# KwangsungKim138/Korean-F5-TTS

Measured on AMD Instinct MI355X. Metric: RTF (audio_sec/wall_sec) F5-TTS Base NFE=16 batch=1, higher is better.
Workload: dtype f16; 1 GPU; C2: F5-TTS Base, 1 utterance/rank/step, prompt 256 + generated 768 mel frames, NFE=16 EPSS, cfg 2.0, sway -1, Vocos decode, mel all_gather when n_gpus>1; global_batch=1, frames=1024, parallelism=dp1, weights=synthetic random-init seed 0

## Files before the change

### korean-f5-tts_amd/csrc/gemm2.h

```cpp
#pragma once
#include "gemm.h"


namespace f5 {

template <int N> __device__ __forceinline__ void wait_vmcnt() { asm volatile("s_waitcnt vmcnt(%0)" ::"n"(N) : "memory"); }

__device__ __forceinline__ void glds16(const void* gsrc, char* lds_dst) {
    __builtin_amdgcn_global_load_lds((const __attribute__((address_space(1))) void*)gsrc,
                                     (__attribute__((address_space(3))) void*)lds_dst, 16, 0, 0);
}

__device__ __forceinline__ void lds_read_b128_asm(u32x4& dst, unsigned addr) {
    asm volatile("ds_read_b128 %0, %1" : "=v"(dst) : "v"(addr));
}
template <int N> __device__ __forceinline__ void wait_lgkm(u32x4& a) { asm volatile("s_waitcnt lgkmcnt(%1)" : "+v"(a) : "n"(N > 15 ? 15 : N)); }
template <int N> __device__ __forceinline__ void wait_lgkm(u32x4& a, u32x4& b) {
    asm volatile("s_waitcnt lgkmcnt(%2)" : "+v"(a), "+v"(b) : "n"(N > 15 ? 15 : N));
}
template <int N> __device__ __forceinline__ void wait_lgkm(u32x4& a, u32x4& b, u32x4& c) {
    asm volatile("s_waitcnt lgkmcnt(%3)" : "+v"(a), "+v"(b), "+v"(c) : "n"(N > 15 ? 15 : N));
}
template <int N> __device__ __forceinline__ void wait_lgkm(u32x4& a, u32x4& b, u32x4& c, u32x4& d) {
    asm volatile("s_waitcnt lgkmcnt(%4)" : "+v"(a), "+v"(b), "+v"(c), "+v"(d) : "n"(N > 15 ? 15 : N));
}
template <int N> __device__ __forceinline__ void wait_lgkm(u32x4& a, u32x4& b, u32x4& c, u32x4& d, u32x4& e) {
    asm volatile("s_waitcnt lgkmcnt(%5)" : "+v"(a), "+v"(b), "+v"(c), "+v"(d), "+v"(e) : "n"(N > 15 ? 15 : N));
}

template <int R, int MI, int NJ, int KK, int I>
__device__ __forceinline__ void wait_row_ct(u32x4 (&af)[2][MI], u32x4 (&wf)[2][NJ]) {
    constexpr int idx = KK * (MI + NJ) + NJ + I;
    constexpr int allow = R - 1 - idx;
    if constexpr (I == 0) {
        if constexpr (NJ == 1) wait_lgkm<allow>(af[KK][0], wf[KK][0]);
        else if constexpr (NJ == 2) wait_lgkm<allow>(af[KK][0], wf[KK][0], wf[KK][1]);
        else if constexpr (NJ == 3) wait_lgkm<allow>(af[KK][0], wf[KK][0], wf[KK][1], wf[KK][2]);
        else wait_lgkm<allow>(af[KK][0], wf[KK][0], wf[KK][1], wf[KK][2], wf[KK][3]);
    } else {
        wait_lgkm<allow>(af[KK][I]);
    }
}
template <int R, int MI, int NJ>
__device__ __forceinline__ void wait_row(int kk, int i, u32x4 (&af)[2][MI], u32x4 (&wf)[2][NJ]) {
#define F5_WR(KK, I) if (kk == KK && i == I) { if constexpr (I < MI) wait_row_ct<R, MI, NJ, KK, I>(af, wf); }
    F5_WR(0, 0) F5_WR(0, 1) F5_WR(0, 2) F5_WR(0, 3) F5_WR(0, 4) F5_WR(0, 5) F5_WR(0, 6) F5_WR(0, 7)
    F5_WR(1, 0) F5_WR(1, 1) F5_WR(1, 2) F5_WR(1, 3) F5_WR(1, 4) F5_WR(1, 5) F5_WR(1, 6) F5_WR(1, 7)
#undef F5_WR
}

typedef __attribute__((ext_vector_type(2))) float f32x2_t;
typedef __attribute__((ext_vector_type(2))) _Float16 f16x2_t;
__device__ __forceinline__ void split8_f16(const u32x4& c0, const u32x4& c1, f16x8& hi, f16x8& lo) {
    const f32x4 x0 = __builtin_bit_cast(f32x4, c0), x1 = __builtin_bit_cast(f32x4, c1);
#pragma unroll
    for (int p = 0; p < 4; ++p) {
        const f32x2_t v = p < 2 ? f32x2_t{x0[2 * p], x0[2 * p + 1]} : f32x2_t{x1[2 * p - 4], x1[2 * p - 3]};
        const f16x2_t h = __builtin_convertvector(v, f16x2_t);
        const f32x2_t r = v - __builtin_convertvector(h, f32x2_t);
        const f16x2_t l = __builtin_convertvector(r, f16x2_t);
        hi[2 * p] = h[0]; hi[2 * p + 1] = h[1];
        lo[2 * p] = l[0]; lo[2 * p + 1] = l[1];
    }
}
__device__ __forceinline__ void tie(u32x4& a) { asm volatile("" : "+v"(a)); }

struct GemmConv { int tpt = 0, dil = 0, half = 0, m_base = 0; };

template <typename T, int BM, int BN, int WM, int WN, int NS, typename Epi, int MODE = 0>
__device__ __forceinline__ void gemm_tn_glds_body(char* smem, const T* __restrict__ A, int lda, const T* __restrict__ W,
                                                  int ldw, int M, int N, int K, const Epi& epi, int xa, int xb,
                                                  const int* __restrict__ m_limit, const GemmConv cv = GemmConv{}) {
    constexpr int NW = WM * WN;
    constexpr int KT = GEMM_ROW_BYTES / sizeof(T);
    constexpr int EPC = 16 / sizeof(T);
    constexpr int TM = BM / WM, TN = BN / WN;
    constexpr int MI = TM / 16, NJ = TN / 16;
    constexpr int STAGE = (BM + BN) * GEMM_ROW_BYTES;
    constexpr int RG_A = BM / 8, RG_W = BN / 8;
    constexpr int LA = RG_A / NW, LW = RG_W / NW;
    static_assert(RG_A % NW == 0 && RG_W % NW == 0, "tile rows must split evenly over the waves");
    constexpr int L = LA + LW;

    const int tid = threadIdx.x, lane = tid & 63;
    const int wave = __builtin_amdgcn_readfirstlane(tid >> 6);
    const int wr = wave / WN, wc = wave % WN;
    int tile_m = blockIdx.y, tile_n = blockIdx.x;
    if (m_limit) {
        const int tiles_n = gridDim.x;
        const int bid = blockIdx.y * tiles_n + blockIdx.x;
        const int idx = bid >> 3;
        tile_m = (idx / tiles_n) * 8 + (bid & 7);
        tile_n = idx % tiles_n;
    } else if (xa > 0) {
        const int tiles_n = gridDim.x;
        const int bid = blockIdx.y * tiles_n + blockIdx.x;
        const int xcd = bid & 7, idx = bid >> 3;
        const int rects_n = tiles_n / xb;
        const int per_rect = xa * xb;
        const int rect = xcd + 8 * (idx / per_rect), in = idx % per_rect;
        tile_m = (rect / rects_n) * xa + in / xb;
        tile_n = (rect % rects_n) * xb + in % xb;
    }
    const int m0 = tile_m * BM, n0 = tile_n * BN;
    if (m_limit) {
        M = min(M, __builtin_amdgcn_readfirstlane(*m_limit));
        if (m0 >= M) return;
    }
    const int nkt = K / KT;
    bool trj[NJ];
    int nt = 0;
#pragma unroll
    for (int j = 0; j < NJ; ++j) {
        trj[j] = Epi::kTransposes && epi.tile_transposed(n0 + (wave % WN) * TN + j * 16);
        nt += trj[j] ? 1 : 0;
    }
    nt = __builtin_amdgcn_readfirstlane(nt);

    const int lr = lane >> 3, lc = (lane & 7) ^ lr;
    const T* asrc[LA];
    const T* wsrc[LW];
#pragma unroll
    for (int i = 0; i < LA; ++i) {
        const int row = min(m0 + (wave + i * NW) * 8 + lr, M - 1);
        asrc[i] = A + (size_t)row * lda + lc * EPC;
    }
#pragma unroll
    for (int i = 0; i < LW; ++i) {
        const int row = min(n0 + (wave + i * NW) * 8 + lr, N - 1);
        wsrc[i] = W + (size_t)row * ldw + lc * EPC;
    }
    auto issue_piece = [&](int p, long akoff, int koff, char* base) {
        if (p < LA) glds16(asrc[p] + akoff, base + (wave + p * NW) * 1024);
        else glds16(wsrc[p - LA] + koff, base + BM * GEMM_ROW_BYTES + (wave + (p - LA) * NW) * 1024);
    };
    auto issue = [&](int kt, int stage) {
        if (kt >= nkt) return;
        char* base = smem + stage * STAGE;
        const int koff = kt * KT;
        long akoff = koff;
        if (cv.tpt > 0) {
            const int tap = kt / cv.tpt;
            akoff = (long)(tap - cv.half) * cv.dil * lda + (long)(kt - tap * cv.tpt) * KT;
        }
#pragma unroll
        for (int p = 0; p < L; ++p) issue_piece(p, akoff, koff, base);
    };
    auto wait_tiles = [&](int tiles) {
        if (tiles >= NS - 2) wait_vmcnt<(NS - 2) * L>();
        else if (NS >= 4 && tiles == NS - 3) wait_vmcnt<(NS >= 4 ? NS - 3 : 0) * L>();
        else if (NS >= 5 && tiles == NS - 4) wait_vmcnt<(NS >= 5 ? NS - 4 : 0) * L>();
        else wait_vmcnt<0>();
// ... 40 lines not shown
        if (any_tr) {
#pragma unroll
            for (int i = 0; i < MI; ++i) {
                const int m = min(mw + i * 16 + g * 4, M - 1);
                trc[i] = epi.trow(m + cv.m_base, M + cv.m_base);
            }
#pragma unroll
            for (int j = 0; j < NJ; ++j) tcc[j] = epi.tcol(min(nw + j * 16 + l15, N - 1));
        }
    };
#pragma unroll
    for (int t = 0; t < NS - 1; ++t) issue(t, t);
    if (EARLY) epilogue_setup();

    __builtin_amdgcn_s_waitcnt(0xC07F);
    auto kloop = [&](auto ntc) {
        constexpr int NT = decltype(ntc)::value;
        constexpr int R = 2 * (MI + NJ);
        auto tile = [&](int stage) {
            u32x4 af[2][MI], wf[2][NJ];
            const unsigned sbu = (unsigned)(stage * STAGE) + lds_base;
#pragma unroll
            for (int kk = 0; kk < 2; ++kk) {
                const unsigned co = kk ? c1 : c0;
                lds_read_b128_asm(af[kk][0], sbu + a_row_off + co);
#pragma unroll
                for (int j = 0; j < NJ; ++j) lds_read_b128_asm(wf[kk][j], sbu + w_row_off + j * 16 * GEMM_ROW_BYTES + co);
#pragma unroll
                for (int i = 1; i < MI; ++i) lds_read_b128_asm(af[kk][i], sbu + a_row_off + i * 16 * GEMM_ROW_BYTES + co);
            }
            if constexpr (MODE == 3 || MODE >= 5) {
#pragma unroll
                for (int i = 0; i < MI; ++i) {
                    __builtin_amdgcn_sched_barrier(0);
                    wait_row<R, MI, NJ>(1, i, af, wf);
                    tie(af[0][i]);
                    if (i == 0) {
#pragma unroll
                        for (int j = 0; j < NJ; ++j) tie(wf[0][j]);
                    }
                    f16x8 ah, al;
                    if constexpr (MODE == 5) { ah = __builtin_bit_cast(f16x8, af[0][i]); al = __builtin_bit_cast(f16x8, af[1][i]); }
                    else split8_f16(af[0][i], af[1][i], ah, al);
#pragma unroll
                    for (int term = (MODE == 6 ? 1 : MODE == 7 ? 2 : 0); term < 3; ++term) {
#pragma unroll
                        for (int j = 0; j < NJ; ++j) {
                            const f16x8 w = __builtin_bit_cast(f16x8, wf[term == 0 ? 1 : 0][j]);
                            const f16x8 a = term == 1 ? al : ah;
                            if (j < NJ - NT) acc[i][j] = __builtin_amdgcn_mfma_f32_16x16x32_f16(w, a, acc[i][j], 0, 0, 0);
                            else acc[i][j] = __builtin_amdgcn_mfma_f32_16x16x32_f16(a, w, acc[i][j], 0, 0, 0);
                        }
                    }
                }
                return;
            }
#pragma unroll
            for (int kk = 0; kk < 2; ++kk) {
#pragma unroll
                for (int i = 0; i < MI; ++i) {
                    __builtin_amdgcn_sched_barrier(0);
                    wait_row<R, MI, NJ>(kk, i, af, wf);
#pragma unroll
                    for (int j = 0; j < NJ; ++j) {
                        if (j < NJ - NT) acc[i][j] = Mma<T>::run(wf[kk][j], af[kk][i], acc[i][j]);
                        else acc[i][j] = Mma<T>::run(af[kk][i], wf[kk][j], acc[i][j]);
                    }
                }
            }
        };
        int stage = 0;
        {
            for (int kt = 0; kt < nkt; ++kt) {
                if (MODE != 2) wait_tiles(nkt - 1 - kt);
                __builtin_amdgcn_s_barrier();
                int pf = stage + NS - 1;
                if (pf >= NS) pf -= NS;
                if (MODE != 2) issue(kt + NS - 1, pf);
                if (MODE != 1) tile(stage);
                stage = stage + 1 == NS ? 0 : stage + 1;
            }
        }
    };
    if constexpr (Epi::kTransposes) {
        constexpr bool MIXED = (BN % 64) != 0 || BN == 192;
        if (nt == 0) kloop(std::integral_constant<int, 0>{});
        else if (nt == NJ) kloop(std::integral_constant<int, NJ>{});
        else if constexpr (MIXED && NJ >= 2) {
            if (nt == 1) kloop(std::integral_constant<int, 1>{});
            else if constexpr (NJ >= 3) {
                if (nt == 2) kloop(std::integral_constant<int, 2>{});
                else if constexpr (NJ >= 4) kloop(std::integral_constant<int, 3>{});
            }
        }
    } else {
        kloop(std::integral_constant<int, 0>{});
    }

    if (MODE == 4 && K > 0) {
        float sink = 0.f;
#pragma unroll
        for (int i = 0; i < MI; ++i)
#pragma unroll
            for (int j = 0; j < NJ; ++j) sink += acc[i][j][0] + acc[i][j][1] + acc[i][j][2] + acc[i][j][3];
        if (sink == 1234.5678f && lda < 0) *reinterpret_cast<volatile float*>(smem) = sink;
        return;
    }
    if (!EARLY) epilogue_setup();
    __builtin_amdgcn_s_waitcnt(0x0F70);
#pragma unroll
    for (int j = 0; j < NJ; ++j) {
        const int n = nw + j * 16 + g * 4;
        if (trj[j] || n >= N) continue;
#pragma unroll
        for (int i = 0; i < MI; ++i)
            if (mw + i * 16 + l15 < M) epi.store(rc[i], cc[j], acc[i][j], pre[i][j]);
    }
    if (any_tr) {
#pragma unroll
        for (int j = 0; j < NJ; ++j) {
            const int n = nw + j * 16 + l15;
            if (!trj[j] || n >= N) continue;
#pragma unroll
            for (int i = 0; i < MI; ++i)
                if (mw + i * 16 + g * 4 < M) epi.tstore(trc[i], tcc[j], acc[i][j]);
        }
    }
}

template <typename T, int BM, int BN, int WM, int WN, int NS, typename Epi, int MODE = 0>
__global__ __launch_bounds__(WM* WN * 64) void gemm_tn_glds_kernel(const T* __restrict__ A, int lda,
                                                                   const T* __restrict__ W, int ldw, int M, int N, int K,
                                                                   Epi epi, int xa, int xb, const int* __restrict__ m_limit,
                                                                   const GemmConv cv) {
    extern __shared__ __attribute__((aligned(16))) char smem[];
    gemm_tn_glds_body<T, BM, BN, WM, WN, NS, Epi, MODE>(smem, A, lda, W, ldw, M, N, K, epi, xa, xb, m_limit, cv);
}

inline int& xcd_mode() { static int m = 1; return m; }
inline void pick_xcd_rect(int tiles_m, int tiles_n, int* xa, int* xb) {
    *xa = *xb = 0;
    if (!xcd_mode()) return;
    long best = -1;
    for (int a = 1; a <= tiles_m && a <= 16; ++a) {
        if (tiles_m % a) continue;
        for (int b = 1; b <= tiles_n && b <= 32; ++b) {
            if (tiles_n % b) continue;
            const long rects = (long)(tiles_m / a) * (tiles_n / b);
            if (rects % 8) continue;
            const int area = a * b;
            if (area > 64) continue;
            const long score = 1000L * (64 - (area > 32 ? area - 32 : 32 - area)) - 10L * (a + b);
            if (score > best) { best = score; *xa = a; *xb = b; }
        }
    }
    if (*xa * *xb <= 1) *xa = *xb = 0;
}

template <typename T, int BM, int BN, int WM, int WN, int NS, typename Epi, int MODE = 0>
inline hipError_t launch_gemm2_raw(hipStream_t s, const T* A, int lda, const T* W, int ldw, int M, int N, int K,
                                   const Epi& epi, const int* m_limit = nullptr, const GemmConv& cv = GemmConv{}) {
    constexpr int smem = NS * (BM + BN) * GEMM_ROW_BYTES;
    static bool attr_set = false;
    if (!attr_set) {
        hipError_t e = hipFuncSetAttribute(reinterpret_cast<const void*>(&gemm_tn_glds_kernel<T, BM, BN, WM, WN, NS, Epi, MODE>),
                                           hipFuncAttributeMaxDynamicSharedMemorySize, smem);
        if (e != hipSuccess) return e;
        attr_set = true;
    }
    dim3 grid((N + BN - 1) / BN, (M + BM - 1) / BM);
    if (m_limit) grid.y = (grid.y + 7) / 8 * 8;
    int xa = 0, xb = 0;
    if (!m_limit) pick_xcd_rect((int)grid.y, (int)grid.x, &xa, &xb);
    hipLaunchKernelGGL((gemm_tn_glds_kernel<T, BM, BN, WM, WN, NS, Epi, MODE>), grid, dim3(WM * WN * 64), smem, s, A, lda, W,
                       ldw, M, N, K, epi, xa, xb, m_limit, cv);
    return hipGetLastError();
}

template <typename T, int BM, int BN, int WM, int WN, int NS, typename Epi, int MODE = 0>
inline hipError_t launch_gemm2_cfg(hipStream_t s, const T* A, int lda, const T* W, int ldw, int M, int N, int K,
                                   const Epi& epi, const int* m_limit = nullptr, const GemmConv& cv = GemmConv{}) {
    return with_static_act(epi, [&](const auto& e) {
        return launch_gemm2_raw<T, BM, BN, WM, WN, NS, std::decay_t<decltype(e)>, MODE>(s, A, lda, W, ldw, M, N, K, e, m_limit, cv);
    });
}

}
```

### korean-f5-tts_amd/csrc/gemm3.h

```cpp
#pragma once
#include "gemm2.h"

namespace f5 {

template <typename E, typename = void> struct epi_staged : std::false_type {};
template <typename E> struct epi_staged<E, std::void_t<decltype(E::kStaged)>> : std::integral_constant<bool, E::kStaged> {};

template <int OFF> __device__ __forceinline__ void lds_read_b128_off(u32x4& dst, unsigned addr) {
    asm volatile("ds_read_b128 %0, %1 offset:%2" : "=v"(dst) : "v"(addr), "n"(OFF));
}
__device__ __forceinline__ void reg_fence(u32x4& a) { asm volatile("" : "+v"(a)); }

template <typename T, typename Epi, int DIAG = 0>
__global__ __launch_bounds__(512) void gemm_pp_kernel(const T* __restrict__ A, int lda, const T* __restrict__ W, int ldw, int M,
                                                      int N, int K, Epi epi, int xa, int xb, const int* __restrict__ m_limit) {
    extern __shared__ __attribute__((aligned(16))) char smem[];
    constexpr int BM = 256, BN = 256;
    constexpr int KT = GEMM_ROW_BYTES / sizeof(T);
    constexpr int EPC = 16 / sizeof(T);
    constexpr int MI = 8, NJ = 4;
    constexpr int RB = GEMM_ROW_BYTES;
    constexpr int BUF = (BM + BN) * RB;

    const int tid = threadIdx.x, lane = tid & 63;
    const int wave = __builtin_amdgcn_readfirstlane(tid >> 6);
    const int wr = wave >> 2, wc = wave & 3;
    int tile_m = blockIdx.y, tile_n = blockIdx.x;
    if (m_limit) {
        const int tiles_n = gridDim.x;
        const int bid = blockIdx.y * tiles_n + blockIdx.x;
        const int idx = bid >> 3;
        tile_m = (idx / tiles_n) * 8 + (bid & 7);
        tile_n = idx % tiles_n;
    } else if (xa > 0) {
        const int tiles_n = gridDim.x;
        const int bid = blockIdx.y * tiles_n + blockIdx.x;
        const int xcd = bid & 7, idx = bid >> 3;
        const int rects_n = tiles_n / xb;
        const int per_rect = xa * xb;
        const int rect = xcd + 8 * (idx / per_rect), in = idx % per_rect;
        tile_m = (rect / rects_n) * xa + in / xb;
        tile_n = (rect % rects_n) * xb + in % xb;
    }
    const int m0 = tile_m * BM, n0 = tile_n * BN;
    if (m_limit) {
        M = min(M, __builtin_amdgcn_readfirstlane(*m_limit));
        if (m0 >= M) return;
    }
    const int nkt = K / KT;
    const bool transposed = Epi::kTransposes && epi.tile_transposed(n0);

    const int lr = lane >> 3, lc = (lane & 7) ^ lr;
    const T* asrc[2][2];
    const T* bsrc[2][2];
    int adst[2][2], bdst[2][2];
#pragma unroll
    for (int u = 0; u < 2; ++u)
#pragma unroll
        for (int h = 0; h < 2; ++h) {
            const int ar = h * 128 + u * 64 + wave * 8;
            asrc[u][h] = A + (size_t)min(m0 + ar + lr, M - 1) * lda + lc * EPC;
            adst[u][h] = ar * RB;
            const int q = wave + 8 * h;
            const int br = (q >> 2) * 64 + u * 32 + (q & 3) * 8;
            bsrc[u][h] = W + (size_t)min(n0 + br + lr, N - 1) * ldw + lc * EPC;
            bdst[u][h] = (BM + br) * RB;
        }
    auto issue_a = [&](int u, int koff, char* base) {
        glds16(asrc[u][0] + koff, base + adst[u][0]);
        glds16(asrc[u][1] + koff, base + adst[u][1]);
    };
    auto issue_b = [&](int u, int koff, char* base) {
        glds16(bsrc[u][0] + koff, base + bdst[u][0]);
        glds16(bsrc[u][1] + koff, base + bdst[u][1]);
    };

    f32x4 acc[MI][NJ];
#pragma unroll
    for (int i = 0; i < MI; ++i)
#pragma unroll
        for (int j = 0; j < NJ; ++j) acc[i][j] = f32x4{0.f, 0.f, 0.f, 0.f};

    const int l15 = lane & 15, g = lane >> 4, sw = l15 & 7;
    const unsigned lds_base = (unsigned)(size_t)(__attribute__((address_space(3))) char*)smem;
    const unsigned a_row = (wr * 128 + l15) * RB, b_row = (BM + wc * 64 + l15) * RB;
    const unsigned c0 = ((0 + g) ^ sw) * 16, c1 = ((4 + g) ^ sw) * 16;

    issue_a(0, 0, smem);
    issue_b(0, 0, smem);
    issue_b(1, 0, smem);
    issue_a(1, 0, smem);
    __builtin_amdgcn_s_waitcnt(0xC07F);
    wait_vmcnt<0>();
// ... 211 lines not shown
```

### korean-f5-tts_amd/csrc/gemm_dispatch.h

```cpp
#pragma once
#include "gemm3.h"

namespace f5 {

enum GemmCfg { G2_128x128_8W = 2, G2_128x64_8W = 9, G2_64x64_4W = 8, G2_128x192_8W = 10, G2_256x128_8W = 13, G3_256x256_PP = 20 };

inline int pick_cfg_v2(int M, int N, bool allow_v3 = false, float g3_penalty = 0.f) {
    static const int forced = getenv("F5_GEMM_CFG") ? atoi(getenv("F5_GEMM_CFG")) : -1;
    static const int forced_n = getenv("F5_GEMM_CFG_N") ? atoi(getenv("F5_GEMM_CFG_N")) : 0;
    if (forced >= 0 && (forced != G3_256x256_PP || allow_v3) && (forced_n == 0 || forced_n == N)) return forced;
    if (M <= 64) return G2_64x64_4W;
    struct Cand { int id, bm, bn; float t; };
    static const Cand cands[] = {{G3_256x256_PP, 256, 256, 37.0f}, {G2_256x128_8W, 256, 128, 21.0f}, {G2_128x192_8W, 128, 192, 19.3f},
                                 {G2_128x128_8W, 128, 128, 14.5f}, {G2_128x64_8W, 128, 64, 7.3f}, {G2_64x64_4W, 64, 64, 4.0f}};
    int best = G2_64x64_4W;
    float best_cost = 3.0e38f;
    for (const Cand& c : cands) {
        if (c.id == G3_256x256_PP && !allow_v3) continue;
        const long tiles = (long)((M + c.bm - 1) / c.bm) * ((N + c.bn - 1) / c.bn);
        const float cost = (float)((tiles + 255) / 256) * (c.t + (c.id == G3_256x256_PP ? g3_penalty : 0.f));
        if (cost < best_cost) { best_cost = cost; best = c.id; }
    }
    return best;
}

template <typename Epi> inline bool epilogue_streams_residual(const Epi&) { return false; }
inline bool epilogue_streams_residual(const EpiGateRes&) { return true; }

template <typename T, typename Epi>
inline hipError_t launch_gemm_v2(hipStream_t s, const T* A, int lda, const T* W, int ldw, int M, int N, int K,
                                 const Epi& epi, int cfg, const int* ml = nullptr, const GemmConv& cv = GemmConv{}, int split = 0) {
    if constexpr (std::is_same_v<T, float>) {
        if (split == 2) {
            switch (cfg) {
                case G3_256x256_PP:
                    if (cv.tpt == 0 && cv.m_base == 0) return launch_gemm3<T, Epi, 8>(s, A, lda, W, ldw, M, N, K, epi, ml);
                    [[fallthrough]];
                case G2_256x128_8W: return launch_gemm2_cfg<T, 256, 128, 4, 2, 3, Epi, 5>(s, A, lda, W, ldw, M, N, K, epi, ml, cv);
                case G2_128x192_8W: return launch_gemm2_cfg<T, 128, 192, 2, 4, 3, Epi, 5>(s, A, lda, W, ldw, M, N, K, epi, ml, cv);
                case G2_128x128_8W: return launch_gemm2_cfg<T, 128, 128, 2, 4, 4, Epi, 5>(s, A, lda, W, ldw, M, N, K, epi, ml, cv);
                case G2_128x64_8W: return launch_gemm2_cfg<T, 128, 64, 4, 2, 4, Epi, 5>(s, A, lda, W, ldw, M, N, K, epi, ml, cv);
                default: return launch_gemm2_cfg<T, 64, 64, 2, 2, 3, Epi, 5>(s, A, lda, W, ldw, M, N, K, epi, ml, cv);
            }
        }
        if (split) {
            switch (cfg) {
                case G3_256x256_PP:
                case G2_256x128_8W: return launch_gemm2_cfg<T, 256, 128, 4, 2, 3, Epi, 3>(s, A, lda, W, ldw, M, N, K, epi, ml, cv);
                case G2_128x192_8W: return launch_gemm2_cfg<T, 128, 192, 2, 4, 3, Epi, 3>(s, A, lda, W, ldw, M, N, K, epi, ml, cv);
                case G2_128x128_8W: return launch_gemm2_cfg<T, 128, 128, 2, 4, 4, Epi, 3>(s, A, lda, W, ldw, M, N, K, epi, ml, cv);
                case G2_128x64_8W: return launch_gemm2_cfg<T, 128, 64, 4, 2, 4, Epi, 3>(s, A, lda, W, ldw, M, N, K, epi, ml, cv);
                default: return launch_gemm2_cfg<T, 64, 64, 2, 2, 3, Epi, 3>(s, A, lda, W, ldw, M, N, K, epi, ml, cv);
            }
        }
    } else if (split) return hipErrorInvalidValue;
    switch (cfg) {
        case G3_256x256_PP:
            if (cv.tpt == 0 && cv.m_base == 0) return launch_gemm3<T, Epi>(s, A, lda, W, ldw, M, N, K, epi, ml);
            [[fallthrough]];
        case G2_256x128_8W: return launch_gemm2_cfg<T, 256, 128, 4, 2, 3, Epi>(s, A, lda, W, ldw, M, N, K, epi, ml, cv);
        case G2_128x192_8W: return launch_gemm2_cfg<T, 128, 192, 2, 4, 3, Epi>(s, A, lda, W, ldw, M, N, K, epi, ml, cv);
        case G2_128x128_8W: return launch_gemm2_cfg<T, 128, 128, 2, 4, 4, Epi>(s, A, lda, W, ldw, M, N, K, epi, ml, cv);
        case G2_128x64_8W: return launch_gemm2_cfg<T, 128, 64, 4, 2, 4, Epi>(s, A, lda, W, ldw, M, N, K, epi, ml, cv);
        default: return launch_gemm2_cfg<T, 64, 64, 2, 2, 3, Epi>(s, A, lda, W, ldw, M, N, K, epi, ml, cv);
    }
}

template <typename T, typename Epi>
inline hipError_t launch_gemm(hipStream_t s, const T* A, int lda, const T* W, int ldw, int M, int N, int K,
                              const Epi& epi, int force_cfg = -1, const int* m_limit = nullptr, int m_hint = 0,
                              const GemmConv& cv = GemmConv{}, int split = 0) {
    if (M <= 0 || N <= 0) return hipSuccess;
    if (split && (K % (GEMM_ROW_BYTES / (int)sizeof(T)) != 0 || force_cfg == -2)) return hipErrorInvalidValue;
    constexpr int KT = GEMM_ROW_BYTES / (int)sizeof(T);
    if (cv.tpt > 0 && (K % KT != 0 || force_cfg == -2)) return hipErrorInvalidValue;
    const float g3_pen = 0.0f;
    const bool v3_ok = ((sizeof(T) == 2 && !split) || split == 2) && gemm3_epilogue_ok(epi);
    if (K % KT == 0 && force_cfg == -1 && !m_limit && cv.tpt == 0 && v3_ok) {
        const int rem = M % 256, main = M - rem;
        const int cfg_main = (rem > 0 && rem <= 64 && main >= 4096) ? pick_cfg_v2(main, N, true, g3_pen) : -1;
        if (cfg_main == G3_256x256_PP || cfg_main == G2_256x128_8W) {
            hipError_t e = launch_gemm_v2<T, Epi>(s, A, lda, W, ldw, main, N, K, epi, cfg_main, nullptr, GemmConv{}, split);
            if (e != hipSuccess) return e;
            GemmConv tail{};
            tail.m_base = main;
            return launch_gemm_v2<T, Epi>(s, A + (size_t)main * lda, lda, W, ldw, rem, N, K, epi, G2_64x64_4W, nullptr, tail, split);
        }
    }
    if (K % KT == 0 && force_cfg != -2) {
        int cfg = force_cfg >= 0 ? force_cfg : pick_cfg_v2(m_hint > 0 ? m_hint : M, N, v3_ok && cv.tpt == 0, g3_pen);
        if (split == 2 && force_cfg < 0 && cfg == G2_128x64_8W && (long)((M + 63) / 64) * ((N + 63) / 64) <= 512) cfg = G2_64x64_4W;
        return launch_gemm_v2<T, Epi>(s, A, lda, W, ldw, M, N, K, epi, cfg, m_limit, cv, split);
    }
    if (m_limit) return hipErrorInvalidValue;
    return launch_gemm_v1<T, Epi>(s, A, lda, W, ldw, M, N, K, epi);
}

}
```

### korean-f5-tts_amd/csrc/kapi.hip

```cpp
#include <vector>

#include "attn2.h"
#include "convpos.h"
#include "elementwise.h"
#include "gemm_dispatch.h"
#include "internal.h"

using namespace f5;
#define fail f5_fail
#define F5K_BY_PREC(prec, FN, ...) \
    ((prec) == F5_PREC_BF16 ? FN<bf16_t>(__VA_ARGS__) : (prec) == F5_PREC_F16 ? FN<f16_t>(__VA_ARGS__) : FN<float>(__VA_ARGS__))
static bool g_split16 = false;
template <typename T> static hipError_t maybe_split(hipStream_t s, T* w, size_t elems) {
    if constexpr (std::is_same_v<T, float>) {
        if (g_split16) hipLaunchKernelGGL(split_planar_kernel, dim3(ew_blocks((long)(elems / 32))), dim3(256), 0, s, w, (long)(elems / 32));
    }
    return hipGetLastError();
}

template <typename T>
static int gemm_impl(const float* A, const float* W, const float* bias, int act, float* out, int M, int N, int K, int tm,
                     int tn, hipStream_t s) {
    const int Kp = tm > 0 ? round_up(K, 8) : round_up(K, 128 / (int)sizeof(T));
    Scratch<T> a, w;
// ... 257 lines not shown
                    EpiQKV<TO>{q, k, static_cast<TO*>(p.out2), bias, frag.p, p.Nseq, p.Npad, p.H, norm ? 0 : p.pe_heads,
                               norm ? 1.0f : p.q_scale, rowmap.p},
                    p.cfg, ml, split));
    if (norm) {
        const long qrows = (long)p.Bp * p.H * p.Nseq;
        hipLaunchKernelGGL((qknorm_rope_kernel<TO>), dim3((unsigned)((qrows * 16 + 255) / 256)), dim3(256), 0, s, q, k, p.gq, p.gk,
                           p.rope_cos, p.rope_sin, qrows, p.Nseq, p.H, p.pe_heads, p.q_scale, 1e-6f);
        KCHK();
    }
    CHK(copy_f32<TO>(s, p.out0, p.out0_f32, p.n0));
    CHK(copy_f32<TO>(s, p.out1, p.out1_f32, p.n1));
    CHK(copy_f32<TO>(s, p.out2, p.out2_f32, p.n2));
    HIPCHK(hipStreamSynchronize(s));
    return F5_OK;
}

template <typename T>
static int gemm_epi_impl(const float* A, const float* W, const float* bias, int M, int N, int K, const f5k_epi& p, hipStream_t s) {
    const int Kp = round_up(K, GEMM_ROW_BYTES / (int)sizeof(T));
    Scratch<T> a, w;
    HIPCHK(a.alloc((size_t)M * Kp));
    HIPCHK(w.alloc((size_t)N * Kp));
    hipLaunchKernelGGL((cast_pad_kernel<T>), dim3(ew_blocks((long)M * Kp)), dim3(256), 0, s, A, K, M, K, a.p, Kp, M);
    hipLaunchKernelGGL((cast_pad_kernel<T>), dim3(ew_blocks((long)N * Kp)), dim3(256), 0, s, W, K, N, K, w.p, Kp, N);
    KCHK();
    int split = 0;
    if constexpr (std::is_same_v<T, float>) {
        if (g_split16) {
            HIPCHK(maybe_split<T>(s, w.p, (size_t)N * Kp));
            if (p.a_presplit) HIPCHK(maybe_split<T>(s, a.p, (size_t)M * Kp));
            split = p.a_presplit ? 2 : 1;
        }
    }
    Scratch<int> ml;
    if (p.m_limit >= 0) {
        HIPCHK(ml.alloc(1));
        HIPCHK(hipMemcpy(ml.p, &p.m_limit, 4, hipMemcpyHostToDevice));
    }
    Scratch<int> lens;
    switch (p.kind) {
        case F5K_EPI_STORE:
            if (p.out16) {
                if constexpr (sizeof(T) == 2) {
                    CHK(epi_gemm<T>(s, a.p, w.p, Kp, M, N, Kp, EpiStore<T>{static_cast<T*>(p.out0), N, bias, p.act}, p.cfg, ml.p, split));
                    CHK(copy_f32<T>(s, p.out0, p.out0_f32, p.n0));
                }
            } else {
                CHK(epi_gemm<T>(s, a.p, w.p, Kp, M, N, Kp, EpiStore<float>{static_cast<float*>(p.out0), N, bias, p.act, p.planar == 1}, p.cfg,
                                ml.p, split));
                if (p.planar == 2) {
                    hipLaunchKernelGGL(split_planar_kernel, dim3(ew_blocks((long)M * N / 32)), dim3(256), 0, s, static_cast<float*>(p.out0),
                                       (long)M * N / 32);
                    KCHK();
                }
            }
            break;
        case F5K_EPI_GATE_RES:
            if (p.lens_host) {
                HIPCHK(lens.alloc((size_t)p.nlens));
                HIPCHK(hipMemcpy(lens.p, p.lens_host, (size_t)p.nlens * 4, hipMemcpyHostToDevice));
            }
            CHK(epi_gemm<T>(s, a.p, w.p, Kp, M, N, Kp,
                            EpiGateRes{static_cast<float*>(p.out0), p.res, N, bias, p.gate, p.gate_stride, p.rows_per_batch, lens.p}, p.cfg,
                            ml.p, split));
            break;
        default:
            if (p.out16) {
                if constexpr (std::is_same_v<T, float>) CHK((epi_qkv<T, f16_t>(s, a.p, w.p, Kp, M, N, Kp, bias, p, ml.p, split)));
            } else {
                CHK((epi_qkv<T, T>(s, a.p, w.p, Kp, M, N, Kp, bias, p, ml.p, split)));
            }
            break;
    }
    HIPCHK(hipStreamSynchronize(s));
    return F5_OK;
}

extern "C" int f5k_gemm_epi(int32_t prec, const float* A, const float* W, const float* bias, int32_t M, int32_t N, int32_t K,
                            const f5k_epi* p, f5_stream stream) {
    if (!A || !W || !p || !p->out0 || M <= 0 || N <= 0 || K <= 0 || (N % 4)) return fail(F5_EINVAL, "f5k_gemm_epi: bad arguments (N %% 4 == 0)");
    if (prec != F5_PREC_F32 && prec != F5_PREC_F16X3 && prec != F5_PREC_BF16 && prec != F5_PREC_F16)
        return fail(F5_EINVAL, "f5k_gemm_epi: precision must be f32, f16x3, bf16 or f16");
    const int c = p->cfg;
    if (c != -1 && c != G2_128x128_8W && c != G2_64x64_4W && c != G2_128x64_8W && c != G2_128x192_8W && c != G2_256x128_8W && c != G3_256x256_PP)
        return fail(F5_EINVAL, "f5k_gemm_epi: cfg must be -1, 2, 8, 9, 10, 13 or 20");
    if (p->m_limit < -1 || p->m_limit > M) return fail(F5_EINVAL, "f5k_gemm_epi: m_limit must be -1 or 0..M");
    if (p->a_presplit && prec != F5_PREC_F16X3) return fail(F5_EINVAL, "f5k_gemm_epi: a_presplit needs F5_PREC_F16X3");
    const bool op16 = prec == F5_PREC_BF16 || prec == F5_PREC_F16;
    switch (p->kind) {
        case F5K_EPI_STORE:
            if (p->out16 && !op16) return fail(F5_EINVAL, "f5k_gemm_epi: a 16-bit STORE needs a 16-bit operand precision");
            if (p->planar < 0 || p->planar > 2 || (p->planar && (p->out16 || prec != F5_PREC_F16X3 || N % 32)) || (p->planar == 2 && p->m_limit >= 0))
                return fail(F5_EINVAL, "f5k_gemm_epi: planar needs an f32 output under f16x3 and N %% 32 == 0 (planar 2: every row)");
            if (p->act != F5_ACT_NONE && p->act != F5_ACT_GELU_TANH) return fail(F5_EINVAL, "f5k_gemm_epi: act must be none or GELU-tanh");
            break;
        case F5K_EPI_GATE_RES:
            if (p->out16 || p->rows_per_batch <= 0 || !p->res) return fail(F5_EINVAL, "f5k_gemm_epi: GATE_RES needs res and rows_per_batch > 0");
            if (p->lens_host && p->nlens < (M - 1) / p->rows_per_batch + 1) return fail(F5_EINVAL, "f5k_gemm_epi: lens shorter than the batch rows");
            break;
        case F5K_EPI_QKV:
        case F5K_EPI_QKNORM: {
            const bool norm = p->kind == F5K_EPI_QKNORM;
            if (!p->out1 || !p->out2 || !bias || !p->rope_cos || !p->rope_sin || p->H <= 0 || N != 3 * p->H * 64 || p->Nseq <= 0 ||
                p->Npad < p->Nseq || p->Npad % 8 || p->pe_heads < 0 || p->pe_heads > p->H || p->maxpos < p->Nseq || p->Bp <= 0)
                return fail(F5_EINVAL, "f5k_gemm_epi: bad QKV arguments");
            if (p->out16 && op16) return fail(F5_EINVAL, "f5k_gemm_epi: out16 QKV is the f16 output of f32 / f16x3 operands");
            if (norm && (p->out16 || !p->gq || !p->gk || p->row_start_host)) return fail(F5_EINVAL, "f5k_gemm_epi: bad QKNORM arguments");
            if (p->row_start_host) {
                if (p->m_limit != -1 || p->row_start_host[0] != 0 || p->row_start_host[p->Bp] > M)
                    return fail(F5_EINVAL, "f5k_gemm_epi: row_start must start at 0, end <= M and replaces m_limit");
                for (int b = 0; b < p->Bp; ++b) {
                    const int cnt = p->row_start_host[b + 1] - p->row_start_host[b];
                    if (p->row_start_host[b] % 4 || cnt < 0 || cnt > round_up(p->Nseq, 4))
                        return fail(F5_EINVAL, "f5k_gemm_epi: row_start entries must be multiples of 4, at most round_up(Nseq, 4) apart");
                }
            } else if (M != p->Bp * p->Nseq) {
                return fail(F5_EINVAL, "f5k_gemm_epi: M must be Bp * Nseq without row_start");
            }
            break;
        }
        default: return fail(F5_EINVAL, "f5k_gemm_epi: unknown epilogue kind");
    }
    hipStream_t s = (hipStream_t)stream;
    g_split16 = prec == F5_PREC_F16X3;
    const int rc = F5K_BY_PREC(prec, gemm_epi_impl, A, W, bias, M, N, K, *p, s);
    g_split16 = false;
    return rc;
}
```

### korean-f5-tts_amd/csrc/kapi_diag.hip

```cpp
#include <vector>

#include "attn2.h"
#include "convpos.h"
#include "elementwise.h"
#include "gemm_dispatch.h"
#include "internal.h"

using namespace f5;
#define fail f5_fail
#define F5K_BY_PREC(prec, FN, ...) \
    ((prec) == F5_PREC_BF16 ? FN<bf16_t>(__VA_ARGS__) : (prec) == F5_PREC_F16 ? FN<f16_t>(__VA_ARGS__) : FN<float>(__VA_ARGS__))

#include "gemm2.h"
static int g_cold_weights = 0;
static int g_out_bf16 = 0;

template <typename T, typename Epi>
static hipError_t gemm2_dispatch(int cfg, hipStream_t s, const T* A, int lda, const T* W, int ldw, int M, int N, int K,
                                 const Epi& epi) {
    switch (cfg) {
        case 0: return launch_gemm2_cfg<T, 128, 128, 2, 2, 3, Epi>(s, A, lda, W, ldw, M, N, K, epi);
        case 1: return launch_gemm2_cfg<T, 128, 128, 2, 2, 4, Epi>(s, A, lda, W, ldw, M, N, K, epi);
        case 13: return launch_gemm2_cfg<T, 256, 128, 4, 2, 3, Epi>(s, A, lda, W, ldw, M, N, K, epi);
        case 20: return launch_gemm3<T, Epi>(s, A, lda, W, ldw, M, N, K, epi);
        case 420: return launch_gemm3<T, Epi, 4>(s, A, lda, W, ldw, M, N, K, epi);
        case 2: return launch_gemm2_cfg<T, 128, 128, 2, 4, 4, Epi>(s, A, lda, W, ldw, M, N, K, epi);
        case 3: return launch_gemm2_cfg<T, 128, 64, 2, 2, 4, Epi>(s, A, lda, W, ldw, M, N, K, epi);
        case 5: return launch_gemm2_cfg<T, 64, 64, 2, 2, 4, Epi>(s, A, lda, W, ldw, M, N, K, epi);
        case 7: return launch_gemm2_cfg<T, 128, 128, 4, 2, 3, Epi>(s, A, lda, W, ldw, M, N, K, epi);
        case 8: return launch_gemm2_cfg<T, 64, 64, 2, 2, 3, Epi>(s, A, lda, W, ldw, M, N, K, epi);
        case 9: return launch_gemm2_cfg<T, 128, 64, 4, 2, 4, Epi>(s, A, lda, W, ldw, M, N, K, epi);
        case 10: return launch_gemm2_cfg<T, 128, 192, 2, 4, 3, Epi>(s, A, lda, W, ldw, M, N, K, epi);
        case 11: return launch_gemm2_cfg<T, 128, 192, 2, 4, 4, Epi>(s, A, lda, W, ldw, M, N, K, epi);
        case 102: return launch_gemm2_cfg<T, 128, 128, 2, 4, 4, Epi, 1>(s, A, lda, W, ldw, M, N, K, epi);
        case 202: return launch_gemm2_cfg<T, 128, 128, 2, 4, 4, Epi, 2>(s, A, lda, W, ldw, M, N, K, epi);
        case 16: return launch_gemm2_cfg<T, 128, 128, 2, 4, 2, Epi>(s, A, lda, W, ldw, M, N, K, epi);
        case 17: return launch_gemm2_cfg<T, 256, 128, 4, 2, 2, Epi>(s, A, lda, W, ldw, M, N, K, epi);
        case 18: return launch_gemm2_cfg<T, 128, 128, 2, 2, 2, Epi>(s, A, lda, W, ldw, M, N, K, epi);
        case 113: return launch_gemm2_cfg<T, 256, 128, 4, 2, 3, Epi, 1>(s, A, lda, W, ldw, M, N, K, epi);
        case 213: return launch_gemm2_cfg<T, 256, 128, 4, 2, 3, Epi, 2>(s, A, lda, W, ldw, M, N, K, epi);
        case 413: return launch_gemm2_cfg<T, 256, 128, 4, 2, 3, Epi, 4>(s, A, lda, W, ldw, M, N, K, epi);
        case 402: return launch_gemm2_cfg<T, 128, 128, 2, 4, 4, Epi, 4>(s, A, lda, W, ldw, M, N, K, epi);
        case 409: return launch_gemm2_cfg<T, 128, 64, 4, 2, 4, Epi, 4>(s, A, lda, W, ldw, M, N, K, epi);
        default: return hipErrorInvalidValue;
    }
}

template <typename T>
static int gemm2_impl(const float* A, const float* W, const float* bias, int act, float* out, int M, int N, int K, int cfg,
                      int iters, float* avg_us, hipStream_t s) {
    const int Kp = round_up(K, 128 / (int)sizeof(T));
    Scratch<T> a, w;
    HIPCHK(a.alloc((size_t)M * Kp));
    HIPCHK(w.alloc((size_t)N * Kp));
    hipLaunchKernelGGL((cast_pad_kernel<T>), dim3(ew_blocks((long)M * Kp)), dim3(256), 0, s, A, K, M, K, a.p, Kp, M);
    hipLaunchKernelGGL((cast_pad_kernel<T>), dim3(ew_blocks((long)N * Kp)), dim3(256), 0, s, W, K, N, K, w.p, Kp, N);
    KCHK();
    HIPCHK(gemm2_dispatch<T>(cfg, s, a.p, Kp, w.p, Kp, M, N, Kp, EpiStore<float>{out, N, bias, act}));
    if (iters > 0 && avg_us) {
        const bool cold = g_cold_weights != 0;
        const size_t wbytes = (size_t)N * Kp * sizeof(T);
        const int ncopy = cold ? (int)std::min<size_t>(64, (320u << 20) / wbytes + 1) : 1;
        Scratch<T> wc;
        if (cold) {
            HIPCHK(wc.alloc((size_t)ncopy * N * Kp));
            for (int c = 0; c < ncopy; ++c)
                HIPCHK(hipMemcpyAsync(wc.p + (size_t)c * N * Kp, w.p, wbytes, hipMemcpyDeviceToDevice, s));
        }
        hipEvent_t e0, e1;
        HIPCHK(hipEventCreate(&e0));
        HIPCHK(hipEventCreate(&e1));
        for (int i = 0; cold && i < ncopy; ++i)
            HIPCHK(gemm2_dispatch<T>(cfg, s, a.p, Kp, wc.p + (size_t)(i % ncopy) * N * Kp, Kp, M, N, Kp, EpiStore<float>{out, N, bias, act}));
        HIPCHK(hipEventRecord(e0, s));
        for (int i = 0; i < iters; ++i) {
            const T* wp = cold ? wc.p + (size_t)(i % ncopy) * N * Kp : w.p;
            if (g_out_bf16)
                HIPCHK(gemm2_dispatch<T>(cfg, s, a.p, Kp, wp, Kp, M, N, Kp, EpiStore<bf16_t>{reinterpret_cast<bf16_t*>(out), N, bias, act}));
            else
                HIPCHK(gemm2_dispatch<T>(cfg, s, a.p, Kp, wp, Kp, M, N, Kp, EpiStore<float>{out, N, bias, act}));
        }
        HIPCHK(hipEventRecord(e1, s));
        HIPCHK(hipEventSynchronize(e1));
        float ms = 0.f;
        HIPCHK(hipEventElapsedTime(&ms, e0, e1));
        *avg_us = ms * 1000.f / iters;
        (void)hipEventDestroy(e0);
        (void)hipEventDestroy(e1);
    }
    HIPCHK(hipStreamSynchronize(s));
    return F5_OK;
}

extern "C" int f5x_set_xcd_mode(int32_t on) { xcd_mode() = on; return 0; }
extern "C" int f5x_set_attn_variant(int32_t v) { attn2_variant() = v; return 0; }
extern "C" int f5x_set_cold_weights(int32_t on) { g_cold_weights = on; return 0; }
extern "C" int f5x_set_out_bf16(int32_t on) { g_out_bf16 = on; return 0; }
extern "C" int f5x_gemm2(int32_t prec, const float* A, const float* W, const float* bias, int32_t act, float* out, int32_t M,
                         int32_t N, int32_t K, int32_t cfg, int32_t iters, float* avg_us, f5_stream stream) {
    if (!A || !W || !out || M <= 0 || N <= 0 || K <= 0 || (N % 4)) return fail(F5_EINVAL, "f5x_gemm2: bad arguments");
    hipStream_t s = (hipStream_t)stream;
    return F5K_BY_PREC(prec, gemm2_impl, A, W, bias, act, out, M, N, K, cfg, iters, avg_us, s);
}


extern "C" int f5x_block_gemm_time(int32_t M, int32_t cfg, int32_t iters, float* us4, f5_stream stream) {
    if (M <= 0 || M % 1024 || iters <= 0 || !us4) return fail(F5_EINVAL, "f5x_block_gemm_time: M must be a multiple of 1024");
    hipStream_t s = (hipStream_t)stream;
    typedef bf16_t T;
    const int D = 1024, F = 2048, N = 1024, ncopy = 8;
    const int H = getenv("F5X_QKV_H") ? atoi(getenv("F5X_QKV_H")) : 16;
    const int PE = getenv("F5X_QKV_PE") ? atoi(getenv("F5X_QKV_PE")) : 1;
    Scratch<T> xn, ao, ffh, q, k, vt, wqkv, wout, wff1, wff2;
    Scratch<float> x, bias, gate, rope, rnd;
    HIPCHK(xn.alloc((size_t)M * D)); HIPCHK(ao.alloc((size_t)M * D)); HIPCHK(ffh.alloc((size_t)M * F));
    HIPCHK(q.alloc((size_t)M * D * 3 / 2)); HIPCHK(k.alloc((size_t)M * D * 3 / 2)); HIPCHK(vt.alloc((size_t)M * D));
// ... 297 lines not shown
```

Before: 237.8 audio_sec/wall_sec.

## Add one-wave-per-SIMD 4-wave GEMM with interleaved LDS reads and DMA pipeline

Adds a new 4-wave (2x2) GEMM k-loop for 16-bit operands. Each MFMA gap carries one ds_read with an immediate offset and one LDS-DMA piece, double-buffering the fragment registers across k halves, and the kernel gets launch bounds allowing two blocks per CU. The config picker gains 128x128 and 128x64 four-wave candidates with slightly lower cost estimates, enabled for M between 1024 and 4096 in f16/bf16 non-split GEMMs. The aim is better overlap of LDS reads, global-to-LDS copies and MFMA than the 8-wave kernels achieve. The costs are more register pressure and complexity, and a possible loss of latency hiding from fewer waves.

After: 233.8 audio_sec/wall_sec. 1.7% lower.

```diff
diff --git a/korean-f5-tts_amd/csrc/gemm2.h b/korean-f5-tts_amd/csrc/gemm2.h
--- a/korean-f5-tts_amd/csrc/gemm2.h
+++ b/korean-f5-tts_amd/csrc/gemm2.h
@@ -49,6 +49,17 @@
 #undef F5_WR
 }
 
+template <int OFF> __device__ __forceinline__ void lds_read_b128_off(u32x4& dst, unsigned addr) {
+    static_assert(OFF >= 0 && OFF < 65536, "ds_read offset field is 16 bits");
+    asm volatile("ds_read_b128 %0, %1 offset:%2" : "=v"(dst) : "v"(addr), "n"(OFF));
+}
+template <typename F, int... I> __device__ __forceinline__ void static_for_impl(F&& f, std::integer_sequence<int, I...>) {
+    (f(std::integral_constant<int, I>{}), ...);
+}
+template <int N, typename F> __device__ __forceinline__ void static_for(F&& f) {
+    static_for_impl(f, std::make_integer_sequence<int, N>{});
+}
+
 typedef __attribute__((ext_vector_type(2))) float f32x2_t;
 typedef __attribute__((ext_vector_type(2))) _Float16 f16x2_t;
 __device__ __forceinline__ void split8_f16(const u32x4& c0, const u32x4& c1, f16x8& hi, f16x8& lo) {
@@ -67,7 +78,7 @@
 
 struct GemmConv { int tpt = 0, dil = 0, half = 0, m_base = 0; };
 
-template <typename T, int BM, int BN, int WM, int WN, int NS, typename Epi, int MODE = 0>
+template <typename T, int BM, int BN, int WM, int WN, int NS, typename Epi, int MODE = 0, int PIPE = 0>
 __device__ __forceinline__ void gemm_tn_glds_body(char* smem, const T* __restrict__ A, int lda, const T* __restrict__ W,
                                                   int ldw, int M, int N, int K, const Epi& epi, int xa, int xb,
                                                   const int* __restrict__ m_limit, const GemmConv cv = GemmConv{}) {
@@ -274,7 +285,93 @@
             }
         }
     };
-    if constexpr (Epi::kTransposes) {
+    auto kloop4 = [&](auto ntc) {
+        constexpr int NT = decltype(ntc)::value;
+        constexpr int NR = MI + NJ, NM = MI * NJ;
+        static_assert(NR <= NM && L <= NM, "one read / one LDS-DMA piece per MFMA gap");
+        static_assert(NS >= 3 && (NS - 2) * L < 64, "ring depth");
+        u32x4 af[2][MI], wf[2][NJ];
+        const unsigned a_off[2] = {lds_base + a_row_off + c0, lds_base + a_row_off + c1};
+        const unsigned w_off[2] = {lds_base + w_row_off + c0, lds_base + w_row_off + c1};
+        auto read = [&](auto rc_, auto sc_, unsigned ab, unsigned wb) {
+            constexpr int r = decltype(rc_)::value, S = decltype(sc_)::value;
+            if constexpr (r == 0) lds_read_b128_off<0>(af[S][0], ab);
+            else if constexpr (r <= NJ) lds_read_b128_off<(r - 1) * 16 * GEMM_ROW_BYTES>(wf[S][r - 1], wb);
+            else lds_read_b128_off<(r - NJ) * 16 * GEMM_ROW_BYTES>(af[S][r - NJ], ab);
+        };
+        auto phase = [&](auto cc_, auto rd_, auto dm_, unsigned sb_next, long akoff, int koff, char* dbase) {
+            constexpr int C = decltype(cc_)::value;
+            constexpr bool RD = decltype(rd_)::value, DM = decltype(dm_)::value;
+            const unsigned ab = a_off[1 - C] + sb_next, wb = w_off[1 - C] + sb_next;
+            static_for<MI>([&](auto ic_) {
+                constexpr int i = decltype(ic_)::value;
+                constexpr int ahead = RD ? (i * NJ < NR ? i * NJ : NR) : 0;
+                __builtin_amdgcn_sched_barrier(0);
+                wait_lgkm<MI - 1 - i + ahead>(af[C][i]);
+                if constexpr (i == 0) {
+#pragma unroll
+                    for (int j = 0; j < NJ; ++j) tie(wf[C][j]);
+                }
+                static_for<NJ>([&](auto jc_) {
+                    constexpr int j = decltype(jc_)::value, m = i * NJ + j;
+                    if constexpr (j < NJ - NT) acc[i][j] = Mma<T>::run(wf[C][j], af[C][i], acc[i][j]);
+                    else acc[i][j] = Mma<T>::run(af[C][i], wf[C][j], acc[i][j]);
+                    if constexpr (RD && m < NR) read(std::integral_constant<int, m>{}, std::integral_constant<int, 1 - C>{}, ab, wb);
+                    if constexpr (DM && m >= NM - L) issue_piece(m - (NM - L), akoff, koff, dbase);
+                    __builtin_amdgcn_sched_barrier(0);
+                });
+            });
+        };
+        auto wait_tiles4 = [&](int tiles) {
+            if (NS >= 6 && tiles >= 4) wait_vmcnt<(NS >= 6 ? 4 : 0) * L>();
+            else if (NS >= 5 && tiles >= 3) wait_vmcnt<(NS >= 5 ? 3 : 0) * L>();
+            else if (NS >= 4 && tiles >= 2) wait_vmcnt<(NS >= 4 ? 2 : 0) * L>();
+            else if (tiles >= 1) wait_vmcnt<L>();
+            else wait_vmcnt<0>();
+        };
+        constexpr std::integral_constant<int, 0> S0{};
+        constexpr std::integral_constant<int, 1> S1{};
+        constexpr std::true_type YES{};
+        constexpr std::false_type NO{};
+        wait_tiles4(min(NS - 2, nkt - 1));
+        __builtin_amdgcn_s_barrier();
+        static_for<NR>([&](auto rc_) { read(rc_, S0, a_off[0], w_off[0]); });
+        int stage = 0, kt = 0;
+        for (; kt + NS - 1 < nkt; ++kt) {
+            phase(S0, YES, NO, (unsigned)(stage * STAGE), 0L, 0, smem);
+            wait_vmcnt<(NS - 3) * L>();
+            __builtin_amdgcn_s_barrier();
+            const int pf = stage == 0 ? NS - 1 : stage - 1;
+            stage = stage + 1 == NS ? 0 : stage + 1;
+            const int kn = kt + NS - 1;
+            const int koff = kn * KT;
+            phase(S1, YES, YES, (unsigned)(stage * STAGE), (long)koff, koff, smem + pf * STAGE);
+        }
+        for (; kt + 1 < nkt; ++kt) {
+            phase(S0, YES, NO, (unsigned)(stage * STAGE), 0L, 0, smem);
+            wait_tiles4(nkt - 2 - kt);
+            __builtin_amdgcn_s_barrier();
+            stage = stage + 1 == NS ? 0 : stage + 1;
+            phase(S1, YES, NO, (unsigned)(stage * STAGE), 0L, 0, smem);
+        }
+        phase(S0, YES, NO, (unsigned)(stage * STAGE), 0L, 0, smem);
+        phase(S1, NO, NO, 0u, 0L, 0, smem);
+    };
+    if constexpr (PIPE != 0) {
+        static_assert(MODE == 0 || MODE == 4, "the one-wave-per-SIMD loop has no split-operand / floor modes");
+        static_assert(WM == 2 && WN == 2 && sizeof(T) == 2, "one wave per SIMD, 16-bit operands");
+        static_assert(TN % 32 == 0 && NJ <= 6, "orientation patterns below");
+        if constexpr (Epi::kTransposes) {
+            if (nt == 0) kloop4(std::integral_constant<int, 0>{});
+            else if (nt == NJ) kloop4(std::integral_constant<int, NJ>{});
+            else if constexpr (NJ == 6) {
+                if (nt == 2) kloop4(std::integral_constant<int, 2>{});
+                else kloop4(std::integral_constant<int, 4>{});
+            }
+        } else {
+            kloop4(std::integral_constant<int, 0>{});
+        }
+    } else if constexpr (Epi::kTransposes) {
         constexpr bool MIXED = (BN % 64) != 0 || BN == 192;
         if (nt == 0) kloop(std::integral_constant<int, 0>{});
         else if (nt == NJ) kloop(std::integral_constant<int, NJ>{});
@@ -320,13 +417,13 @@
     }
 }
 
-template <typename T, int BM, int BN, int WM, int WN, int NS, typename Epi, int MODE = 0>
-__global__ __launch_bounds__(WM* WN * 64) void gemm_tn_glds_kernel(const T* __restrict__ A, int lda,
+template <typename T, int BM, int BN, int WM, int WN, int NS, typename Epi, int MODE = 0, int PIPE = 0>
+__global__ __launch_bounds__(WM* WN * 64, PIPE && BN <= 128 ? 2 : 1) void gemm_tn_glds_kernel(const T* __restrict__ A, int lda,
                                                                    const T* __restrict__ W, int ldw, int M, int N, int K,
                                                                    Epi epi, int xa, int xb, const int* __restrict__ m_limit,
                                                                    const GemmConv cv) {
     extern __shared__ __attribute__((aligned(16))) char smem[];
-    gemm_tn_glds_body<T, BM, BN, WM, WN, NS, Epi, MODE>(smem, A, lda, W, ldw, M, N, K, epi, xa, xb, m_limit, cv);
+    gemm_tn_glds_body<T, BM, BN, WM, WN, NS, Epi, MODE, PIPE>(smem, A, lda, W, ldw, M, N, K, epi, xa, xb, m_limit, cv);
 }
 
 inline int& xcd_mode() { static int m = 1; return m; }
@@ -349,13 +446,13 @@
     if (*xa * *xb <= 1) *xa = *xb = 0;
 }
 
-template <typename T, int BM, int BN, int WM, int WN, int NS, typename Epi, int MODE = 0>
+template <typename T, int BM, int BN, int WM, int WN, int NS, typename Epi, int MODE = 0, int PIPE = 0>
 inline hipError_t launch_gemm2_raw(hipStream_t s, const T* A, int lda, const T* W, int ldw, int M, int N, int K,
                                    const Epi& epi, const int* m_limit = nullptr, const GemmConv& cv = GemmConv{}) {
     constexpr int smem = NS * (BM + BN) * GEMM_ROW_BYTES;
     static bool attr_set = false;
     if (!attr_set) {
-        hipError_t e = hipFuncSetAttribute(reinterpret_cast<const void*>(&gemm_tn_glds_kernel<T, BM, BN, WM, WN, NS, Epi, MODE>),
+        hipError_t e = hipFuncSetAttribute(reinterpret_cast<const void*>(&gemm_tn_glds_kernel<T, BM, BN, WM, WN, NS, Epi, MODE, PIPE>),
                                            hipFuncAttributeMaxDynamicSharedMemorySize, smem);
         if (e != hipSuccess) return e;
         attr_set = true;
@@ -364,16 +461,16 @@
     if (m_limit) grid.y = (grid.y + 7) / 8 * 8;
     int xa = 0, xb = 0;
     if (!m_limit) pick_xcd_rect((int)grid.y, (int)grid.x, &xa, &xb);
-    hipLaunchKernelGGL((gemm_tn_glds_kernel<T, BM, BN, WM, WN, NS, Epi, MODE>), grid, dim3(WM * WN * 64), smem, s, A, lda, W,
+    hipLaunchKernelGGL((gemm_tn_glds_kernel<T, BM, BN, WM, WN, NS, Epi, MODE, PIPE>), grid, dim3(WM * WN * 64), smem, s, A, lda, W,
                        ldw, M, N, K, epi, xa, xb, m_limit, cv);
     return hipGetLastError();
 }
 
-template <typename T, int BM, int BN, int WM, int WN, int NS, typename Epi, int MODE = 0>
+template <typename T, int BM, int BN, int WM, int WN, int NS, typename Epi, int MODE = 0, int PIPE = 0>
 inline hipError_t launch_gemm2_cfg(hipStream_t s, const T* A, int lda, const T* W, int ldw, int M, int N, int K,
                                    const Epi& epi, const int* m_limit = nullptr, const GemmConv& cv = GemmConv{}) {
     return with_static_act(epi, [&](const auto& e) {
-        return launch_gemm2_raw<T, BM, BN, WM, WN, NS, std::decay_t<decltype(e)>, MODE>(s, A, lda, W, ldw, M, N, K, e, m_limit, cv);
+        return launch_gemm2_raw<T, BM, BN, WM, WN, NS, std::decay_t<decltype(e)>, MODE, PIPE>(s, A, lda, W, ldw, M, N, K, e, m_limit, cv);
     });
 }
 
diff --git a/korean-f5-tts_amd/csrc/gemm3.h b/korean-f5-tts_amd/csrc/gemm3.h
--- a/korean-f5-tts_amd/csrc/gemm3.h
+++ b/korean-f5-tts_amd/csrc/gemm3.h
@@ -6,9 +6,6 @@
 template <typename E, typename = void> struct epi_staged : std::false_type {};
 template <typename E> struct epi_staged<E, std::void_t<decltype(E::kStaged)>> : std::integral_constant<bool, E::kStaged> {};
 
-template <int OFF> __device__ __forceinline__ void lds_read_b128_off(u32x4& dst, unsigned addr) {
-    asm volatile("ds_read_b128 %0, %1 offset:%2" : "=v"(dst) : "v"(addr), "n"(OFF));
-}
 __device__ __forceinline__ void reg_fence(u32x4& a) { asm volatile("" : "+v"(a)); }
 
 template <typename T, typename Epi, int DIAG = 0>
diff --git a/korean-f5-tts_amd/csrc/gemm_dispatch.h b/korean-f5-tts_amd/csrc/gemm_dispatch.h
--- a/korean-f5-tts_amd/csrc/gemm_dispatch.h
+++ b/korean-f5-tts_amd/csrc/gemm_dispatch.h
@@ -3,20 +3,30 @@
 
 namespace f5 {
 
-enum GemmCfg { G2_128x128_8W = 2, G2_128x64_8W = 9, G2_64x64_4W = 8, G2_128x192_8W = 10, G2_256x128_8W = 13, G3_256x256_PP = 20 };
+enum GemmCfg { G2_128x128_8W = 2, G2_128x64_8W = 9, G2_64x64_4W = 8, G2_128x192_8W = 10, G2_256x128_8W = 13, G3_256x256_PP = 20,
+               G4_128x128_4W = 24, G4_128x64_4W = 25, G4_128x192_4W = 26 };
+inline int cfg_8wave(int cfg) {
+    return cfg == G4_128x128_4W ? G2_128x128_8W : cfg == G4_128x64_4W ? G2_128x64_8W : cfg == G4_128x192_4W ? G2_128x192_8W : cfg;
+}
 
-inline int pick_cfg_v2(int M, int N, bool allow_v3 = false, float g3_penalty = 0.f) {
+constexpr int G4_MIN_ROWS = 1024, G4_MAX_ROWS = 4096;
+constexpr int G4_NS_128x192 = 3, G4_NS_128x128 = 4, G4_NS_128x64 = 5;
+
+inline int pick_cfg_v2(int M, int N, bool allow_v3 = false, float g3_penalty = 0.f, bool allow_4w = false) {
     static const int forced = getenv("F5_GEMM_CFG") ? atoi(getenv("F5_GEMM_CFG")) : -1;
     static const int forced_n = getenv("F5_GEMM_CFG_N") ? atoi(getenv("F5_GEMM_CFG_N")) : 0;
     if (forced >= 0 && (forced != G3_256x256_PP || allow_v3) && (forced_n == 0 || forced_n == N)) return forced;
+    static const bool no_4w = getenv("F5_GEMM_4W") && atoi(getenv("F5_GEMM_4W")) == 0;
     if (M <= 64) return G2_64x64_4W;
     struct Cand { int id, bm, bn; float t; };
     static const Cand cands[] = {{G3_256x256_PP, 256, 256, 37.0f}, {G2_256x128_8W, 256, 128, 21.0f}, {G2_128x192_8W, 128, 192, 19.3f},
-                                 {G2_128x128_8W, 128, 128, 14.5f}, {G2_128x64_8W, 128, 64, 7.3f}, {G2_64x64_4W, 64, 64, 4.0f}};
+                                 {G4_128x128_4W, 128, 128, 13.9f}, {G2_128x128_8W, 128, 128, 14.5f},
+                                 {G4_128x64_4W, 128, 64, 6.9f}, {G2_128x64_8W, 128, 64, 7.3f}, {G2_64x64_4W, 64, 64, 4.0f}};
     int best = G2_64x64_4W;
     float best_cost = 3.0e38f;
     for (const Cand& c : cands) {
         if (c.id == G3_256x256_PP && !allow_v3) continue;
+        if (c.id != cfg_8wave(c.id) && (!allow_4w || no_4w || M < G4_MIN_ROWS || M > G4_MAX_ROWS)) continue;
         const long tiles = (long)((M + c.bm - 1) / c.bm) * ((N + c.bn - 1) / c.bn);
         const float cost = (float)((tiles + 255) / 256) * (c.t + (c.id == G3_256x256_PP ? g3_penalty : 0.f));
         if (cost < best_cost) { best_cost = cost; best = c.id; }
@@ -31,6 +41,7 @@
 inline hipError_t launch_gemm_v2(hipStream_t s, const T* A, int lda, const T* W, int ldw, int M, int N, int K,
                                  const Epi& epi, int cfg, const int* ml = nullptr, const GemmConv& cv = GemmConv{}, int split = 0) {
     if constexpr (std::is_same_v<T, float>) {
+        cfg = cfg_8wave(cfg);
         if (split == 2) {
             switch (cfg) {
                 case G3_256x256_PP:
@@ -54,6 +65,15 @@
             }
         }
     } else if (split) return hipErrorInvalidValue;
+    if (cv.tpt > 0) cfg = cfg_8wave(cfg);
+    if constexpr (sizeof(T) == 2) {
+        switch (cfg) {
+            case G4_128x192_4W: return launch_gemm2_cfg<T, 128, 192, 2, 2, G4_NS_128x192, Epi, 0, 1>(s, A, lda, W, ldw, M, N, K, epi, ml, cv);
+            case G4_128x128_4W: return launch_gemm2_cfg<T, 128, 128, 2, 2, G4_NS_128x128, Epi, 0, 1>(s, A, lda, W, ldw, M, N, K, epi, ml, cv);
+            case G4_128x64_4W: return launch_gemm2_cfg<T, 128, 64, 2, 2, G4_NS_128x64, Epi, 0, 1>(s, A, lda, W, ldw, M, N, K, epi, ml, cv);
+            default: break;
+        }
+    }
     switch (cfg) {
         case G3_256x256_PP:
             if (cv.tpt == 0 && cv.m_base == 0) return launch_gemm3<T, Epi>(s, A, lda, W, ldw, M, N, K, epi, ml);
@@ -88,7 +108,7 @@
         }
     }
     if (K % KT == 0 && force_cfg != -2) {
-        int cfg = force_cfg >= 0 ? force_cfg : pick_cfg_v2(m_hint > 0 ? m_hint : M, N, v3_ok && cv.tpt == 0, g3_pen);
+        int cfg = force_cfg >= 0 ? force_cfg : pick_cfg_v2(m_hint > 0 ? m_hint : M, N, v3_ok && cv.tpt == 0, g3_pen, sizeof(T) == 2 && !split);
         if (split == 2 && force_cfg < 0 && cfg == G2_128x64_8W && (long)((M + 63) / 64) * ((N + 63) / 64) <= 512) cfg = G2_64x64_4W;
         return launch_gemm_v2<T, Epi>(s, A, lda, W, ldw, M, N, K, epi, cfg, m_limit, cv, split);
     }
diff --git a/korean-f5-tts_amd/csrc/kapi.hip b/korean-f5-tts_amd/csrc/kapi.hip
--- a/korean-f5-tts_amd/csrc/kapi.hip
+++ b/korean-f5-tts_amd/csrc/kapi.hip
@@ -363,8 +363,11 @@
     if (prec != F5_PREC_F32 && prec != F5_PREC_F16X3 && prec != F5_PREC_BF16 && prec != F5_PREC_F16)
         return fail(F5_EINVAL, "f5k_gemm_epi: precision must be f32, f16x3, bf16 or f16");
     const int c = p->cfg;
-    if (c != -1 && c != G2_128x128_8W && c != G2_64x64_4W && c != G2_128x64_8W && c != G2_128x192_8W && c != G2_256x128_8W && c != G3_256x256_PP)
-        return fail(F5_EINVAL, "f5k_gemm_epi: cfg must be -1, 2, 8, 9, 10, 13 or 20");
+    if (c != -1 && c != G2_128x128_8W && c != G2_64x64_4W && c != G2_128x64_8W && c != G2_128x192_8W && c != G2_256x128_8W && c != G3_256x256_PP &&
+        c != G4_128x128_4W && c != G4_128x64_4W && c != G4_128x192_4W)
+        return fail(F5_EINVAL, "f5k_gemm_epi: cfg must be -1, 2, 8, 9, 10, 13, 20 or 24, 25, 26");
+    if (c != cfg_8wave(c) && (prec != F5_PREC_BF16 && prec != F5_PREC_F16))
+        return fail(F5_EINVAL, "f5k_gemm_epi: the 4-wave kernels (cfg 24, 25, 26) take 16-bit operands");
     if (p->m_limit < -1 || p->m_limit > M) return fail(F5_EINVAL, "f5k_gemm_epi: m_limit must be -1 or 0..M");
     if (p->a_presplit && prec != F5_PREC_F16X3) return fail(F5_EINVAL, "f5k_gemm_epi: a_presplit needs F5_PREC_F16X3");
     const bool op16 = prec == F5_PREC_BF16 || prec == F5_PREC_F16;
diff --git a/korean-f5-tts_amd/csrc/kapi_diag.hip b/korean-f5-tts_amd/csrc/kapi_diag.hip
--- a/korean-f5-tts_amd/csrc/kapi_diag.hip
+++ b/korean-f5-tts_amd/csrc/kapi_diag.hip
@@ -32,6 +32,12 @@
         case 9: return launch_gemm2_cfg<T, 128, 64, 4, 2, 4, Epi>(s, A, lda, W, ldw, M, N, K, epi);
         case 10: return launch_gemm2_cfg<T, 128, 192, 2, 4, 3, Epi>(s, A, lda, W, ldw, M, N, K, epi);
         case 11: return launch_gemm2_cfg<T, 128, 192, 2, 4, 4, Epi>(s, A, lda, W, ldw, M, N, K, epi);
+        case 24: case 25: case 26:
+            if constexpr (sizeof(T) == 2) return launch_gemm_v2<T, Epi>(s, A, lda, W, ldw, M, N, K, epi, cfg);
+            else return hipErrorInvalidValue;
+        case 424:
+            if constexpr (sizeof(T) == 2) return launch_gemm2_cfg<T, 128, 128, 2, 2, G4_NS_128x128, Epi, 4, 1>(s, A, lda, W, ldw, M, N, K, epi);
+            else return hipErrorInvalidValue;
         case 102: return launch_gemm2_cfg<T, 128, 128, 2, 4, 4, Epi, 1>(s, A, lda, W, ldw, M, N, K, epi);
         case 202: return launch_gemm2_cfg<T, 128, 128, 2, 4, 4, Epi, 2>(s, A, lda, W, ldw, M, N, K, epi);
         case 16: return launch_gemm2_cfg<T, 128, 128, 2, 4, 2, Epi>(s, A, lda, W, ldw, M, N, K, epi);
```
